# NJU-3DV/Relightable3DGaussian

Measured on AMD Instinct MI355X. Metric: train iters/s, synthetic lego-like 800x800, 300000 Gaussians (stage-2 hot path), higher is better.
Workload: dtype f32; 1 GPU; stage-2 train iteration (fused glue kernels + one-launch Adam): shading fwd/bwd (K=64) + rasterize fwd (S=16) + loss + rasterize bwd + Adam; 1 view/rank/step, 300000 Gaussians, 800x800, num_rendered~1755023; parallelism=dp1

## Files before the change

### include/r3dg_hip.h

```cpp
#ifndef R3DG_HIP_H
#define R3DG_HIP_H

#include <stddef.h>
#include <stdint.h>

#ifdef __cplusplus
extern "C" {
#endif

#define R3DG_OK 0
#define R3DG_EINVAL (-1)
#define R3DG_EHIP (-2)
#define R3DG_EALLOC (-3)

typedef void* (*r3dg_alloc_fn)(void* user, size_t bytes);

const char* r3dg_last_error(void);
int r3dg_release_scratch(void);
int r3dg_version(void);

int r3dg_max_features_forward(void);
int r3dg_max_features_backward(void);

size_t r3dg_geometry_state_bytes(int P);
// ... 293 lines not shown
int r3dg_densify_accumulate(void* stream, int P, const float* d_viewspace_grad, const float* d_normal_grad,
                            const int32_t* d_radii, const float* d_weights, float* d_xyz_gradient_accum,
                            float* d_normal_gradient_accum, float* d_denom, float* d_weights_accum,
                            float* d_max_radii2D,
                            const float* d_skip_flag);

typedef struct r3dg_densify_config {
    int32_t mode;
    int32_t n_split;
    float grad_threshold, grad_normal_threshold, min_opacity, weights_threshold;
    float dense_size, world_size_limit, split_divisor, max_screen_size;
} r3dg_densify_config;

size_t r3dg_densify_temp_bytes(int P);
int r3dg_densify_plan(void* stream, int P, const r3dg_densify_config* config, const float* d_scaling_raw,
                      const float* d_opacity_raw, const float* d_xyz_gradient_accum,
                      const float* d_normal_gradient_accum, const float* d_denom, const float* d_weights_accum,
                      const float* d_max_radii2D, int32_t* d_src_row, int32_t* d_kind, int32_t* d_counts, void* d_temp);

#define R3DG_DENSIFY_MAX_GROUPS 24
#define R3DG_DENSIFY_ROLE_COPY 0
#define R3DG_DENSIFY_ROLE_XYZ 1
#define R3DG_DENSIFY_ROLE_SCALING 2
typedef struct r3dg_densify_group {
    const float* src_param;
    const float* src_exp_avg;
    const float* src_exp_avg_sq;
    float* dst_param;
    float* dst_exp_avg;
    float* dst_exp_avg_sq;
    uint32_t row_floats, role;
} r3dg_densify_group;
int r3dg_densify_gather(void* stream, int rows_out, const int32_t* d_src_row, const int32_t* d_kind, int n_groups,
                        const r3dg_densify_group* groups, const float* d_xyz, const float* d_scaling_raw,
                        const float* d_rotation_raw, const float* d_normal_table, float split_divisor);

int r3dg_reset_opacity(void* stream, int P, float* d_opacity_raw, float* d_exp_avg, float* d_exp_avg_sq);

size_t r3dg_knn_temp_bytes(int P);
int r3dg_knn_dist2(void* stream, int P, const float* d_points, float* d_mean_dist2, void* d_temp);

size_t r3dg_bvh_build_temp_bytes(int P);
int r3dg_bvh_build(void* stream, int P, int32_t* d_nodes, float* d_aabbs, int64_t* d_morton, void* d_temp);
int r3dg_bvh_trace_opacity(void* stream, int64_t num_rays, int num_gaussians, const int32_t* d_nodes, const float* d_aabbs,
                           const float* d_rays_o, const float* d_rays_d, const float* d_means3D,
                           const float* d_covs3D, const float* d_opacities, const float* d_normals,
                           int32_t* d_num_contributes, float* d_rendered_opacity, int32_t* d_stack_overflow);

size_t r3dg_bvh_trace_records_bytes(int num_gaussians);
int r3dg_bvh_pack_traversal(void* stream, int num_gaussians, const int32_t* d_nodes, const float* d_aabbs,
                            const float* d_means3D, const float* d_covs3D, const float* d_opacities,
                            const float* d_normals, void* d_records);
int r3dg_bvh_trace_opacity_packed(void* stream, int64_t num_rays, int num_gaussians, void* d_records, const float* d_rays_o,
                                  const float* d_rays_d, int32_t* d_num_contributes, float* d_rendered_opacity,
                                  int32_t* d_stack_overflow);
int r3dg_bvh_trace_visits(void* stream, int num_gaussians, const void* d_records, uint64_t* node_and_leaf_steps);

int r3dg_bvh_trace_count(void* stream, int64_t num_rays, const int32_t* d_nodes, const float* d_aabbs,
                         const float* d_rays_o, const float* d_rays_d, int32_t* d_num_contributes,
                         int32_t* d_stack_overflow);
int r3dg_bvh_trace_fill(void* stream, int64_t num_rays, const int32_t* d_nodes, const float* d_aabbs,
                        const float* d_rays_o, const float* d_rays_d, const float* d_means3D,
                        const int32_t* d_num_contributes, const int64_t* d_offsets_inclusive, uint64_t* d_keys,
                        int32_t* d_point_list, float* d_position_list, int32_t* d_ray_id_list);

size_t r3dg_sort_temp_bytes(int64_t n);
int r3dg_sort_pairs(void* stream, int64_t n, uint64_t* d_keys_in, uint32_t* d_vals_in, uint64_t* d_keys_out,
                    uint32_t* d_vals_out, int end_bit, void* d_temp);

enum r3dg_option {
    R3DG_OPT_TILE_ORDER = 0,
    R3DG_OPT_CULL,
    R3DG_OPT_TILE_BINNING,
    R3DG_OPT_BINNING_BLOCK_K,
    R3DG_OPT_STAGE_SH_ROWS,
    R3DG_OPT_SHADE_FWD_BLOCKS_PER_CU,
    R3DG_OPT_TRACE_FORMULATION,
    R3DG_OPT_TRACE_REFILL,
    R3DG_OPT_TRACE_NODE_WEIGHT,
    R3DG_OPT_TRACE_LEAF_WEIGHT,
    R3DG_OPT_RESERVE_CUS,
    R3DG_OPT_TRACE_COUNT_VISITS,
    R3DG_OPT_BWD_LEAN,
    R3DG_OPT_COUNT
};
int r3dg_set_option(int option, int value);
int r3dg_get_option(int option, int* value);
void* r3dg_context_create(void);
void r3dg_context_destroy(void* ctx);
int r3dg_context_set_option(void* ctx, int option, int value);
int r3dg_context_make_current(void* ctx, void** previous);
int r3dg_selftest_transpose_reduce(void* stream, int N, int dpp, const float* d_in, float* d_out, int* d_chan,
                                   int* d_owner);

int r3dg_profile_enable(int on);
int r3dg_profile_pause(int paused);
int r3dg_profile_num_stages(void);
const char* r3dg_profile_stage_name(int stage);
int r3dg_profile_read(double* ms_out, int* count_out);

#ifdef __cplusplus
}
#endif
#endif
```

### relightable3dgaussian_amd/_lib.py

```python
import ctypes as C
import threading
import os

_HERE = os.path.dirname(os.path.abspath(__file__))
LIB_PATH = os.environ.get("R3DG_LIB_PATH") or os.path.join(_HERE, "lib", "libr3dg_hip.so")

ALLOC_FN = C.CFUNCTYPE(C.c_void_p, C.c_void_p, C.c_size_t)

_lib = None

_f = C.c_float
_i = C.c_int
_p = C.c_void_p

_SIGNATURES = {
    "r3dg_last_error": (C.c_char_p, []),
    "r3dg_version": (_i, []),
    "r3dg_release_scratch": (_i, []),
    "r3dg_max_features_forward": (_i, []),
    "r3dg_max_features_backward": (_i, []),
    "r3dg_bounded_forward_supported": (_i, [_i, _i]),
    "r3dg_geometry_state_bytes": (C.c_size_t, [_i]),
    "r3dg_image_state_bytes": (C.c_size_t, [_i, _i]),
    "r3dg_binning_state_bytes": (C.c_size_t, [C.c_int64]),
# ... 48 lines not shown
    "r3dg_shade_frs_backward": (_i, [_p, _i, _i] + [_p] * 6 + [_i, _i, _p, _f] + [_p] * 6 + [_i] + [_p] * 10 + [_i, _p]),
    "r3dg_shade_frs_incident_chain": (_i, [_p, _i] + [_p] * 8 + [_f] * 5 + [_i, _f, _p, _i]),
    "r3dg_shade_build_transport": (_i, [_p, _i, _i, _i, _p, _p, _p, _p, _p, _f, _p, _p]),
    "r3dg_shade_forward_transport": (_i, [_p, _i, _i] + [_p] * 9),
    "r3dg_shade_build_split": (_i, [_p, _i, _i] + [_p] * 6 + [_f, _p, _p, _p]),
    "r3dg_shade_env_footprints_bytes": (C.c_size_t, [_i, _i]),
    "r3dg_shade_env_footprints": (_i, [_p, _i, _i, _p, _p]),
    "r3dg_shade_forward_split": (_i, [_p, _i, _i] + [_p] * 11 + [_i, _i, _p]),
    "r3dg_shade_backward": (_i, [_p, _i, _i, _i, _p, _p, _p, _p, _p, _p, _i, _i, _p, _p, _p, _p, _p, _p, _p, _p, _p,
                                 _p, _p]),
    "r3dg_shade_backward_cached": (_i, [_p, _i, _i, _i, _p, _p, _p, _p, _p, _p, _i, _i, _p, _p, _p, _p, _p, _p, _p, _p, _p,
                                        _p, _p, _p, _p, _i]),
    "r3dg_render_equation_forward": (_i, [_p, _i, _i, _i, _i] + [_p] * 8 + [_i] + [_p] * 4),
    "r3dg_render_equation_forward_complex": (_i, [_p, _i, _i, _i, _i] + [_p] * 8 + [_i] + [_p] * 11),
    "r3dg_render_equation_backward": (_i, [_p, _i, _i, _i, _i] + [_p] * 8 + [_i] + [_p] * 11),
    "r3dg_clock_probe": (_i, [_p, _i, _p, _p, C.POINTER(C.c_int)]),
    "r3dg_stage2_activate": (_i, [_p, _i] + [_p] * 17),
    "r3dg_stage2_activate_with": (_i, [_p, _i] + [_p] * 17 + [_i, _p, _p, _p, _i]),
    "r3dg_stage2_pack_features": (_i, [_p, _i] + [_p] * 8),
    "r3dg_stage2_unpack_gradients": (_i, [_p, _i, _p, _p, _f, _p, _p, _p, _p]),
    "r3dg_stage2_activate_backward": (_i, [_p, _i] + [_p] * 24),
    "r3dg_stage2_activate_backward_with": (_i, [_p, _i] + [_p] * 24 + [_i, _i, _p, _p, _p, _f, _p, _p, _i]),
    "r3dg_stage2_loss": (_i, [_p, _i, _i] + [_p] * 8 + [_f, _f, _f] + [_p] * 6 + [_i]),
    "r3dg_stage2_smooth_forward": (_i, [_p, _i, _i] + [_p] * 5 + [_f, _f, _f, _p, _p]),
    "r3dg_stage2_smooth_backward": (_i, [_p, _i, _i] + [_p] * 5 + [_f, _f, _f, _i, _p, _p]),
    "r3dg_stage2_smooth_fused": (_i, [_p, _i, _i] + [_p] * 5 + [_f, _f, _f, _i, _p, _p, _p]),
    "r3dg_stage2_pbr_srgb": (_i, [_p, _i, _i] + [_p] * 5),
    "r3dg_stage2_normals_srgb": (_i, [_p, _i, _i, _p, _f, _f, _f, _f] + [_p] * 8),
    "r3dg_ssim_forward": (_i, [_p, _i, _i, _i, _p, _p, _p, _p]),
    "r3dg_ssim_backward": (_i, [_p, _i, _i, _i, _p, _p, _p, _f, _p]),
    "r3dg_ssim_forward_pair": (_i, [_p, _i, _i, _i] + [_p] * 7),
    "r3dg_ssim_backward_pair": (_i, [_p, _i, _i, _i] + [_p] * 5 + [_f, _f, _p, _p]),
    "r3dg_stage1_pack_features": (_i, [_p, _i, _p, _p, _p, _p]),
    "r3dg_stage1_loss": (_i, [_p, _i, _i] + [_p] * 7 + [_f] * 5 + [_p] * 6),
    "r3dg_stage1_activate_backward": (_i, [_p, _i] + [_p] * 16),
    "r3dg_stage2_env_backward": (_i, [_p, _i, _i, _p, _p, _p, _f, _p, _p, _i]),
    "r3dg_adam_step": (_i, [_p, _i, _p, _f, _f, _f, _i, _f, _p]),
    "r3dg_relight_pack_features": (_i, [_p, _i] + [_p] * 7),
    "r3dg_relight_compose": (_i, [_p, _i, _i, _f, _f, _f, _f, _p, _p, _p, _i, _i] + [_p] * 7),
    "r3dg_densify_accumulate": (_i, [_p, _i] + [_p] * 10),
    "r3dg_densify_temp_bytes": (C.c_size_t, [_i]),
    "r3dg_densify_plan": (_i, [_p, _i] + [_p] * 12),
    "r3dg_densify_gather": (_i, [_p, _i, _p, _p, _i, _p, _p, _p, _p, _p, _f]),
    "r3dg_reset_opacity": (_i, [_p, _i, _p, _p, _p]),
    "r3dg_knn_temp_bytes": (C.c_size_t, [_i]),
    "r3dg_knn_dist2": (_i, [_p, _i, _p, _p, _p]),
    "r3dg_bvh_build_temp_bytes": (C.c_size_t, [_i]),
    "r3dg_bvh_build": (_i, [_p, _i, _p, _p, _p, _p]),
    "r3dg_bvh_trace_opacity": (_i, [_p, C.c_int64, _i, _p, _p, _p, _p, _p, _p, _p, _p, _p, _p, _p]),
    "r3dg_bvh_trace_records_bytes": (C.c_size_t, [_i]),
    "r3dg_bvh_pack_traversal": (_i, [_p, _i] + [_p] * 7),
    "r3dg_bvh_trace_opacity_packed": (_i, [_p, C.c_int64, _i] + [_p] * 6),
    "r3dg_bvh_trace_visits": (_i, [_p, _i, _p, C.POINTER(C.c_uint64)]),
    "r3dg_profile_enable": (_i, [_i]),
    "r3dg_profile_pause": (_i, [_i]),
    "r3dg_profile_num_stages": (_i, []),
    "r3dg_profile_stage_name": (C.c_char_p, [_i]),
    "r3dg_profile_read": (_i, [C.POINTER(C.c_double), C.POINTER(_i)]),
}

EXTRA_SIGNATURES = {}


def lib():
    global _lib
    if _lib is None:
        if not os.path.exists(LIB_PATH):
            raise RuntimeError(
                "libr3dg_hip.so not found at %s -- build it with `python -m relightable3dgaussian_amd.build` "
                "(hipcc, gfx950). There is no CPU fallback." % LIB_PATH)
        import torch
        L = C.CDLL(LIB_PATH)
        sigs = dict(_SIGNATURES)
        sigs.update(EXTRA_SIGNATURES)
        for name, (res, args) in sigs.items():
            fn = getattr(L, name)
            fn.restype = res
            fn.argtypes = args
        _lib = L
    return _lib


OPTIONS = ("TILE_ORDER", "CULL", "TILE_BINNING", "BINNING_BLOCK_K", "STAGE_SH_ROWS", "SHADE_FWD_BLOCKS_PER_CU", "TRACE_FORMULATION",
           "TRACE_REFILL", "TRACE_NODE_WEIGHT", "TRACE_LEAF_WEIGHT", "RESERVE_CUS", "TRACE_COUNT_VISITS", "BWD_LEAN")


def set_option(name, value):
    check(lib().r3dg_set_option(OPTIONS.index(name), int(value)), "set_option(%s)" % name)


_live_lock = threading.Lock()
_live_entries = {}


class OptionContext:

    def __init__(self, **options):
        self._h = lib().r3dg_context_create()
        if self._h is None:
            raise RuntimeError("r3dg_context_create failed")
        self._tls = threading.local()
        for k, v in options.items():
            self.set(k, v)

    def set(self, name, value):
        check(lib().r3dg_context_set_option(self._h, OPTIONS.index(name), int(value)), "context_set_option(%s)" % name)

    def __enter__(self):
        prev = _p()
        check(lib().r3dg_context_make_current(self._h, C.byref(prev)), "context_make_current")
        stack = getattr(self._tls, "prev", None)
        if stack is None:
            stack = self._tls.prev = []
        stack.append(prev.value)
        with _live_lock:
            _live_entries[self._h] = _live_entries.get(self._h, 0) + 1
        return self

    def __exit__(self, *exc):
        check(lib().r3dg_context_make_current(self._tls.prev.pop(), None), "context_make_current")
        with _live_lock:
            n = _live_entries.get(self._h, 0) - 1
            if n > 0:
                _live_entries[self._h] = n
            else:
                _live_entries.pop(self._h, None)
        return False

    def __del__(self):
        try:
            if self._h:
                with _live_lock:
                    busy = _live_entries.get(self._h, 0) > 0
                if not busy:
                    lib().r3dg_context_destroy(self._h)
                self._h = None
        except Exception:
            pass


def get_option(name):
    v = C.c_int(0)
    check(lib().r3dg_get_option(OPTIONS.index(name), C.byref(v)), "get_option(%s)" % name)
    return v.value


def check(status, what):
    if status != 0:
        msg = lib().r3dg_last_error()
        raise RuntimeError("%s failed (%d): %s" % (what, status, msg.decode() if msg else "?"))


def ptr(t):
    if t is None or t.numel() == 0:
        return None
    return t.data_ptr()


def current_stream():
    import torch
    raw = getattr(torch._C, "_cuda_getCurrentRawStream", None)
    if raw is not None:
        return raw(torch._C._cuda_getDevice())
    return torch.cuda.current_stream().cuda_stream


def stream_wait(waiter, signaller):
# ... 23 lines not shown
```

### relightable3dgaussian_amd/csrc/capi_core.hip

```cpp
#include "capi_internal.hpp"

#include <map>
#include <mutex>
#include <new>
#include <tuple>
#include <vector>

namespace r3dg {

static thread_local std::string g_last_error;
void set_error(const std::string& msg) { g_last_error = msg; }

struct OptionRow { int id, def, lo, hi; };
constexpr OptionRow kOptions[] = {
    {R3DG_OPT_TILE_ORDER, 1, 0, 1},
    {R3DG_OPT_CULL, 1, 0, 1},
    {R3DG_OPT_TILE_BINNING, 2, 0, 2},
    {R3DG_OPT_BINNING_BLOCK_K, 2, 1, 4},
    {R3DG_OPT_STAGE_SH_ROWS, 1, 0, 1},
    {R3DG_OPT_SHADE_FWD_BLOCKS_PER_CU, 0, 0, 8},
    {R3DG_OPT_TRACE_FORMULATION, 4, 0, 4},
    {R3DG_OPT_TRACE_REFILL, REFILL_MIN_IDLE, 1, 64},
    {R3DG_OPT_TRACE_NODE_WEIGHT, 1, 1, 15},
    {R3DG_OPT_TRACE_LEAF_WEIGHT, 1, 1, 15},
    {R3DG_OPT_RESERVE_CUS, 0, 0, 128},
    {R3DG_OPT_TRACE_COUNT_VISITS, 0, 0, 1},
    {R3DG_OPT_BWD_LEAN, 1, 0, 1},
};
constexpr bool option_rows_in_enum_order()
{
    for (int i = 0; i < (int)(sizeof(kOptions) / sizeof(kOptions[0])); i++)
        if (kOptions[i].id != i) return false;
    return true;
}
static_assert(sizeof(kOptions) / sizeof(kOptions[0]) == R3DG_OPT_COUNT && option_rows_in_enum_order(),
              "kOptions needs one row per r3dg_option, in the order of the enum");

static bool option_known(int option) { return option >= 0 && option < R3DG_OPT_COUNT; }
static bool option_in_range(int option, int value) { return value >= kOptions[option].lo && value <= kOptions[option].hi; }

struct OptionContext {
    int value[R3DG_OPT_COUNT];
    unsigned int set_mask;
};
static OptionContext g_process_options;
static thread_local const OptionContext* tl_context = nullptr;

int opt(int option)
{
    const OptionContext* c = tl_context;
    if (c != nullptr && ((c->set_mask >> option) & 1u)) return c->value[option];
    return (g_process_options.set_mask >> option) & 1u ? g_process_options.value[option] : kOptions[option].def;
}

namespace {
struct ScratchBuf { void* p = nullptr; size_t cap = 0; };
std::mutex g_scratch_mu;
std::map<std::tuple<int, hipStream_t, int>, ScratchBuf> g_scratch;
}

void* stream_scratch(hipStream_t stream, int slot, size_t bytes)
{
    int dev = 0;
    R3DG_HIP(hipGetDevice(&dev));
    std::lock_guard<std::mutex> lk(g_scratch_mu);
    ScratchBuf& b = g_scratch[std::make_tuple(dev, stream, slot)];
    if (b.cap < bytes) {
        const size_t want = b.p == nullptr ? bytes + bytes / 8 + 4096 : std::max(bytes + 4096, 2 * b.cap);
        if (b.p != nullptr) {
            R3DG_HIP(hipStreamSynchronize(stream));
            R3DG_HIP(hipFree(b.p));
            b.p = nullptr;
            b.cap = 0;
        }
        R3DG_HIP(hipMalloc(&b.p, want));
        b.cap = want;
    }
    return b.p;
}

static void release_all_scratch()
{
    R3DG_HIP(hipDeviceSynchronize());
    {
        std::lock_guard<std::mutex> lk(g_scratch_mu);
        for (auto& kv : g_scratch)
            if (kv.second.p != nullptr) (void)hipFree(kv.second.p);
        g_scratch.clear();
    }
    release_gradient_records();
}

static int g_profiling = 0;
struct EventPair { hipEvent_t a, b; };
static std::vector<EventPair> g_events[ST_COUNT];
static std::mutex g_prof_mutex;

StageTimer::StageTimer(hipStream_t s_, int stage_) : s(s_), stage(stage_), on(g_profiling != 0)
{
    if (on) {
        R3DG_HIP(hipEventCreate(&a));
        R3DG_HIP(hipEventCreate(&b));
        R3DG_HIP(hipEventRecord(a, s));
    }
}
void StageTimer::stop()
{
    if (on) {
        R3DG_HIP(hipEventRecord(b, s));
        std::lock_guard<std::mutex> lk(g_prof_mutex);
// ... 225 lines not shown
```

### relightable3dgaussian_amd/csrc/shading.hip

```cpp
#include "launchers.hpp"
#include <cmath>
#include <cstdlib>
#include <map>
#include <mutex>
#include <stdexcept>
#include <tuple>
#include "wave_reduce.hpp"
#include "shading_math.hpp"

namespace r3dg {

constexpr int SHADE_WAVES = 4;
constexpr int ENV_LDS_MAX = 12288;

__device__ __forceinline__ float fast_acosf(float x)
{
    const float ax = fabsf(x);
    const bool big = ax > 0.5f;
    const float z = big ? 0.5f * (1.0f - ax) : x * x;
    const float s = big ? sqrtf(z) : ax;
    float p = 4.2163199048e-2f;
    p = p * z + 2.4181311049e-2f;
    p = p * z + 4.5470025998e-2f;
    p = p * z + 7.4953002686e-2f;
// ... 1079 lines not shown
                                     const float* normals, const float* viewdirs, const float* incidents, const float* env, int He,
                                     int We, const float* visibility, const float* ray_normals, const float* zsamples,
                                     float uniform_area, const int* invalid_list, int n_invalid, float* out, float* feat)
{
    if (n_invalid <= 0) return;
    const FrsSrc src = {base_color, roughness, normals, viewdirs, ray_normals, nullptr, nullptr, nullptr, visibility, nullptr};
    const size_t smem = ((((size_t)3 * He * We + 3) & ~(size_t)3) + 64 * FRS_LISTED_WAVES) * sizeof(float);
    shade_forward_frs_listed_kernel<<<frs_listed_grid(n_invalid), 64 * FRS_LISTED_WAVES, smem, s>>>(
        n_invalid, invalid_list, K, src, incidents, env, He, We, zsamples, frs_area(uniform_area), out, feat);
    check_launch(s, false, "shade_forward_frs_listed_kernel");
}

const unsigned int* launch_shade_frs_backward_aux(hipStream_t s, int P, const float* g_pbr, const float* g_diff,
                                                  const float* block_absmax, int n_block_absmax, int* gmax_n)
{
    unsigned int* scratch = shade_scratch();
    const unsigned int* gmax = scratch;
    *gmax_n = 1;
    if (block_absmax != nullptr && n_block_absmax > 0) {
        gmax = reinterpret_cast<const unsigned int*>(block_absmax);
        *gmax_n = n_block_absmax;
    } else {
        R3DG_HIP(hipMemsetAsync(scratch, 0, 4, s));
        const int nb = (3 * P + 255) / 256;
        grad_absmax_kernel<<<nb < 256 ? nb : 256, 256, 0, s>>>(3 * P, g_pbr, g_diff, scratch);
    }
    return gmax;
}

void launch_shade_frs_backward_main(hipStream_t s, int P, int K, const float* base_color, const float* roughness,
                                    const float* normals, const float* viewdirs, const float* env, int He, int We,
                                    const float* visibility, float uniform_area, const uint32_t* taps, const float* ray_normals,
                                    const float* tables, const uint8_t* valid, const float* cprime, float* dcp, const float* g_pbr,
                                    const float* g_diff, float* d_base, float* d_rough, float* d_view, float* d_env,
                                    const unsigned int* gmax, int gmax_n)
{
    if (P == 0) return;
    const bool tab_lds = K <= FRS_TAB_LDS_MAX_K;
    const size_t smem = frs_backward_lds_bytes(K, He, We);
    const FrsSrc src = {base_color, roughness, normals, viewdirs, ray_normals, cprime, g_pbr, g_diff, visibility, taps};
    if (tab_lds) {
        const int grid = frs_grid(P, (const void*)shade_backward_frs_kernel<true>, smem);
        shade_backward_frs_kernel<true><<<grid, 64 * FRS_WAVES, smem, s>>>(
            P, K, src, env, He, We, frs_area(uniform_area), tables, valid, d_base, d_rough, d_view, dcp, d_env, gmax, gmax_n);
    } else {
        const int grid = frs_grid(P, (const void*)shade_backward_frs_kernel<false>, smem);
        shade_backward_frs_kernel<false><<<grid, 64 * FRS_WAVES, smem, s>>>(
            P, K, src, env, He, We, frs_area(uniform_area), tables, valid, d_base, d_rough, d_view, dcp, d_env, gmax, gmax_n);
    }
    check_launch(s, false, "shade_backward_frs_kernel");
}

void launch_shade_frs_backward_rotate(hipStream_t s, int P, const float* ray_normals, const float* dcp, float* d_inc,
                                      const uint8_t* valid)
{
    if (P == 0) return;
    frs_rotate_kernel<true><<<(P + 255) / 256, 256, 0, s>>>(P, ray_normals, dcp, d_inc, valid);
    check_launch(s, false, "frs_rotate_kernel");
}

void launch_shade_frs_incident_chain(hipStream_t s, int P, const float* ray_normals, const uint8_t* valid, const float* dcp,
                                     float* d_inc, float* incidents, float* exp_avg, float* exp_avg_sq, float* cprime, float lr,
                                     float lr_tail, float beta1, float beta2, float eps, int step, float grad_scale,
                                     const float* skip_flag, int listed_in_dcprime)
{
    if (P == 0) return;
    const double b1 = 1.0 - pow((double)beta1, (double)step), b2 = 1.0 - pow((double)beta2, (double)step);
    FrsAdam a = {lr, lr_tail, beta1, beta2, eps, (float)b1, (float)(1.0 / sqrt(b2)), grad_scale, 1.f - beta1, 1.f - beta2};
    const size_t lds = 4 * 64 * FRS_CHAIN_LD * sizeof(float);
    frs_incident_chain_kernel<<<(P + 255) / 256, 256, lds, s>>>(P, ray_normals, valid, dcp, d_inc, incidents, exp_avg, exp_avg_sq,
                                                                cprime, a, skip_flag, listed_in_dcprime);
    check_launch(s, false, "frs_incident_chain_kernel");
}

void launch_shade_frs_backward_listed(hipStream_t s, int K, const float* base_color, const float* roughness,
                                      const float* normals, const float* viewdirs, const float* incidents, const float* env, int He,
                                      int We, const float* visibility, const float* ray_normals, const float* zsamples,
                                      float uniform_area, const int* invalid_list, int n_invalid, const float* g_pbr,
                                      const float* g_diff, float* d_base, float* d_rough, float* d_view, float* d_inc, float* d_env,
                                      const unsigned int* gmax, int gmax_n)
{
    if (n_invalid <= 0) return;
    const FrsSrc src = {base_color, roughness, normals, viewdirs, ray_normals, nullptr, g_pbr, g_diff, visibility, nullptr};
    const size_t smem = (3 * (((size_t)3 * He * We + 3) & ~(size_t)3) + 64 * FRS_LISTED_WAVES) * sizeof(float);
    int grid = frs_listed_grid(n_invalid);
    grid = grid > 64 ? 64 + (grid - 64) / 4 : grid;
    if (smem > 65536)
        R3DG_HIP(hipFuncSetAttribute((const void*)shade_backward_frs_listed_kernel, hipFuncAttributeMaxDynamicSharedMemorySize,
                                     (int)smem));
    shade_backward_frs_listed_kernel<<<grid, 64 * FRS_LISTED_WAVES, smem, s>>>(
        n_invalid, invalid_list, K, src, incidents, env, He, We, zsamples, frs_area(uniform_area), d_base, d_rough, d_view, d_inc,
        d_env, gmax, gmax_n);
    check_launch(s, false, "shade_backward_frs_listed_kernel");
}

void launch_shade_build_split(hipStream_t s, int P, int K, const int* perm, const float* normals, const float* incidents,
                              const float* visibility, const float* dirs, const float* zsamples, float uniform_area, float* lt,
                              float* vis_t, float* consts)
{
    if (P == 0) return;
    shade_build_split_kernel<<<(P + 255) / 256, 256, 0, s>>>(P, K, perm, normals, incidents, visibility, dirs, zsamples,
                                                           frs_area(uniform_area), reinterpret_cast<float4*>(lt), vis_t, consts);
    check_launch(s, false, "shade_build_split_kernel");
}

void launch_shade_forward_split(hipStream_t s, int P, int K, const int* perm, const float* base_color, const float* roughness,
                                const float* normals, const float* viewdirs, const float* lt, const float* vis_t,
                                const float* consts, const float* zsamples, const float* tr, const float* env_fp, int He, int We,
                                float* out)
{
    if (P == 0) return;
    const int waves = (P + 63) / 64;
    int parts = (12 * 4 * shade_cus() + waves - 1) / waves;
    parts = parts < 1 ? 1 : (parts > 8 ? 8 : parts);
    int Kp = ((K + parts - 1) / parts + 3) & ~3;
    parts = (K + Kp - 1) / Kp;
    float4* partial = reinterpret_cast<float4*>(stream_scratch(s, 1, (size_t)parts * P * 3 * sizeof(float4)));
    const dim3 grid((P + 255) / 256, parts);
    shade_forward_split_kernel<<<grid, 256, 0, s>>>(P, K, Kp, perm, base_color, roughness, normals, viewdirs,
                                                   reinterpret_cast<const float4*>(lt), vis_t, zsamples, tr,
                                                   reinterpret_cast<const float4*>(env_fp), He, We, partial);
    shade_split_combine_kernel<<<(P + 255) / 256, 256, 0, s>>>(P, K, parts, perm, base_color, partial, consts, out);
    check_launch(s, false, "shade_forward_split_kernel");
}

void launch_shade_env_footprints(hipStream_t s, int He, int We, const float* env, float* fp)
{
    const int n = (He + 1) * (We + 1);
    shade_env_footprints_kernel<<<(n + 255) / 256, 256, 0, s>>>(He, We, env, reinterpret_cast<float4*>(fp));
    check_launch(s, false, "shade_env_footprints_kernel");
}

void launch_shade_build_transport(hipStream_t s, int P, int K, int M, const float* normals, const float* incidents,
                                  const float* visibility, const float* dirs, const float* areas, float uniform_area,
                                  float* radiance_to_transport, float* consts)
{
    if (P == 0) return;
    shade_build_transport_kernel<<<(P + TR_WAVES - 1) / TR_WAVES, 64 * TR_WAVES, 0, s>>>(
        P, K, M, normals, incidents, visibility, dirs, areas, uniform_area, radiance_to_transport, consts);
    check_launch(s, false, "shade_build_transport_kernel");
}

void launch_shade_forward_transport(hipStream_t s, int P, int K, const float* base_color, const float* roughness,
                                    const float* normals, const float* viewdirs, const float* transport, const float* consts,
                                    const float* zsamples, const float* dirs, float* out)
{
    if (P == 0) return;
    shade_forward_transport_kernel<<<(P + TR_WAVES - 1) / TR_WAVES, 64 * TR_WAVES, 0, s>>>(
        P, K, base_color, roughness, normals, viewdirs, transport, consts, zsamples, dirs, out);
    check_launch(s, false, "shade_forward_transport_kernel");
}


}
```

### relightable3dgaussian_amd/csrc/shading_frs.hpp

```cpp
#pragma once
#include "sh_rotation_tables.hpp"

namespace r3dg {

typedef float f32x4 __attribute__((ext_vector_type(4)));

constexpr int FRS_WAVES = 4;
constexpr int FRS_G = 16;
constexpr float FRS_MAX_DEFECT = 2e-5f;
constexpr int FRS_TAB_LDS_MAX_K = 128;

__device__ __forceinline__ void frs_rotation(const float n0, const float n1, const float n2, float (&R)[9])
{
    const float v1 = -n1, v2 = n0, cp = fmaxf(n2 + 1.f, 1e-7f);
    const bool regular = n2 + 1.f > 0.f;
    R[0] = regular ? 1.f + (-v2 * v2) / cp : -1.f;
    R[1] = regular ? v1 * v2 / cp : 0.f;
    R[2] = regular ? v2 : 0.f;
    R[3] = R[1];
    R[4] = regular ? 1.f + (-v1 * v1) / cp : -1.f;
    R[5] = regular ? -v1 : 0.f;
    R[6] = regular ? -v2 : 0.f;
    R[7] = regular ? v1 : 0.f;
    R[8] = regular ? 1.f + (-v2 * v2 - v1 * v1) / cp : -1.f;
// ... 798 lines not shown
            o[1] = make_float4(dcq[1][1], dcq[2][1], dcq[0][2], dcq[1][2]);
            o[2] = make_float4(dcq[2][2], dcq[0][3], dcq[1][3], dcq[2][3]);
        }
    }
    if (fixed) {
        __syncthreads();
        const float inv = 1.0f / fx_scale;
        for (int i = threadIdx.x; i < 3 * ntexel; i += blockDim.x) {
            const long long v64 = s_denv[i];
            if (v64 != 0) atomicAdd(&d_env[i], (float)((double)v64 * (double)inv));
        }
    }
}

constexpr int FRS_LISTED_WAVES = 4;

__device__ __forceinline__ float frs_listed_record(int lane, int g, const FrsSrc& p, const float* __restrict__ incidents)
{
    const float* q = incidents + (size_t)g * 48 + lane;
    if (lane >= 48) q = p.base_color + 3 * (size_t)g + (lane - 48);
    if (lane == 51) q = p.roughness + g;
    if (lane >= 52) q = p.normals + 3 * (size_t)g + (lane - 52);
    if (lane >= 55) q = p.viewdirs + 3 * (size_t)g + (lane - 55);
    if (lane >= 58) q = p.ray_normals + 3 * (size_t)g + (lane - 58);
    return lane < 61 ? *q : 0.f;
}

__device__ __forceinline__ void frs_listed_direction(const float (&R)[9], const float* __restrict__ zsamples, int k, float& dx,
                                                     float& dy, float& dz)
{
    const float zx = zsamples[3 * k], zy = zsamples[3 * k + 1], zz = zsamples[3 * k + 2];
    dx = R[0] * zx + R[1] * zy + R[2] * zz; dy = R[3] * zx + R[4] * zy + R[5] * zz; dz = R[6] * zx + R[7] * zy + R[8] * zz;
    const float len = fmaxf(sqrtf(dx * dx + dy * dy + dz * dz), 1e-12f);
    dx /= len; dy /= len; dz /= len;
}

__global__ void __launch_bounds__(64 * FRS_LISTED_WAVES)
shade_forward_frs_listed_kernel(int n_list, const int* __restrict__ list, int K, FrsSrc src,
                                const float* __restrict__ incidents, const float* __restrict__ env, int He, int We,
                                const float* __restrict__ zsamples, float uniform_area, float* __restrict__ out,
                                float* __restrict__ feat)
{
    extern __shared__ __attribute__((aligned(16))) float s_mem[];
    float* s_env = s_mem;
    const int ntex = 3 * He * We;
    for (int i = threadIdx.x; i < ntex; i += blockDim.x) s_env[i] = env[i];
    __syncthreads();
    const int lane = threadIdx.x & 63, wave = threadIdx.x >> 6;
    float* u = s_mem + ((ntex + 3) & ~3) + wave * 64;
    const float invK = 1.0f / (float)K;
    for (int i = blockIdx.x * FRS_LISTED_WAVES + wave; i < n_list; i += gridDim.x * FRS_LISTED_WAVES) {
        const int g = __builtin_amdgcn_readfirstlane(list[i]);
        u[lane] = frs_listed_record(lane, g, src, incidents);
        GaussFwd G;
        gauss_setup(G, u);
        float R[9];
        frs_rotation(u[58], u[59], u[60], R);
        float v[8] = {0.f, 0.f, 0.f, 0.f, 0.f, 0.f, 0.f, 0.f};
        for (int kb = 0; kb < K; kb += 64) {
            const int k = kb + lane, kc = min(k, K - 1);
            float dx, dy, dz;
            frs_listed_direction(R, zsamples, kc, dx, dy, dz);
            const float vis = src.visibility[(size_t)g * K + kc];
            SampleFwd s;
            shade_sample<true>(s, G, u, 16, dx, dy, dz, vis, uniform_area, nullptr, s_env, nullptr, He, We);
            if (k < K) {
#pragma unroll
                for (int c = 0; c < 3; c++) {
                    v[c] += (G.base[c] / kPi + s.spec) * s.transport[c];
                    v[3 + c] += s.transport[c];
                }
                v[6] += vis;
            }
        }
        const float r = transpose_reduce<8, true>(v);
        const int ch = transposed_channel<8>(lane);
        if (transposed_owner<8>(lane) && ch < 7) {
            out[(size_t)g * SHADE_NOUT + (ch < 6 ? ch : 18)] = r * invK;
            if (feat != nullptr) feat[(size_t)g * 16 + (ch < 3 ? 2 + ch : 9 + ch)] = r * invK;
        }
    }
}

__global__ void __launch_bounds__(64 * FRS_LISTED_WAVES)
shade_backward_frs_listed_kernel(int n_list, const int* __restrict__ list, int K, FrsSrc src,
                                 const float* __restrict__ incidents, const float* __restrict__ env, int He, int We,
                                 const float* __restrict__ zsamples, float uniform_area, float* __restrict__ d_base,
                                 float* __restrict__ d_rough, float* __restrict__ d_view, float* __restrict__ d_inc,
                                 float* __restrict__ d_env, const unsigned int* __restrict__ gmax_bits, int gmax_n)
{
    extern __shared__ __attribute__((aligned(16))) float s_mem[];
    const int ntex = 3 * He * We, ntex4 = (ntex + 3) & ~3;
    float* s_env = s_mem;
    long long* s_denv = reinterpret_cast<long long*>(s_mem + ntex4);
    const unsigned int gmax_word = wave_gmax_bits(gmax_bits, gmax_n);
    const float gmax = __uint_as_float(gmax_word);
    const bool fixed = gmax_usable(gmax_word);
    const float fx_scale = fixed ? 34359738368.0f / gmax : 0.f;
    const float fx_clamp = gmax * 8192.0f;
    for (int i = threadIdx.x; i < ntex; i += blockDim.x) {
        s_env[i] = env[i];
        s_denv[i] = 0;
    }
    __syncthreads();
    const int lane = threadIdx.x & 63, wave = threadIdx.x >> 6;
    float* u = s_mem + 3 * ntex4 + wave * 64;
    const float invK = 1.0f / (float)K;
    for (int i = blockIdx.x * FRS_LISTED_WAVES + wave; i < n_list; i += gridDim.x * FRS_LISTED_WAVES) {
        const int g = __builtin_amdgcn_readfirstlane(list[i]);
        u[lane] = frs_listed_record(lane, g, src, incidents);
        GaussFwd G;
        gauss_setup(G, u);
        float R[9];
        frs_rotation(u[58], u[59], u[60], R);
        float gp[3], gd[3];
#pragma unroll
        for (int c = 0; c < 3; c++) {
            gp[c] = src.g_pbr[3 * (size_t)g + c] * invK;
            gd[c] = src.g_diff[3 * (size_t)g + c] * invK;
        }
        float acc[64];
#pragma unroll
        for (int f = 0; f < 64; f++) acc[f] = 0.f;
        for (int kb = 0; kb < K; kb += 64) {
            const int k = kb + lane, kc = min(k, K - 1);
            float dx, dy, dz;
            frs_listed_direction(R, zsamples, kc, dx, dy, dz);
            const float vis = src.visibility[(size_t)g * K + kc];
            SampleFwd s;
            shade_sample<true>(s, G, u, 16, dx, dy, dz, vis, k < K ? uniform_area : 0.f, nullptr, s_env, nullptr, He, We);
            float gspec = 0.f, dlin[3], dl[3];
#pragma unroll
            for (int c = 0; c < 3; c++) {
                const float dT = gp[c] * (G.base[c] / kPi + s.spec) + gd[c];
                gspec += gp[c] * s.transport[c];
                acc[48 + c] += gp[c] * s.transport[c] / kPi;
                dlin[c] = dT * s.area_ndi;
                dl[c] = s.shsum[c] >= 0.f ? dlin[c] : 0.f;
            }
            if (s.vis != 0.f && s.area_ndi != 0.f) {
                const float ev[3] = {dlin[0] * s.vis, dlin[1] * s.vis, dlin[2] * s.vis};
                const double scale_d = (double)fx_scale;
#pragma unroll
                for (int tt = 0; tt < 4; tt++) {
                    if (s.taps.idx[tt] < 0) continue;
#pragma unroll
                    for (int c = 0; c < 3; c++) {
                        const float val = ev[c] * s.taps.w[tt];
                        if (fixed) {
                            const float cl = __builtin_amdgcn_fmed3f(val, -fx_clamp, fx_clamp);
                            const double dsum = __builtin_fma((double)cl, scale_d, 6755399441055744.0);
                            const unsigned long long bits = (unsigned long long)__double_as_longlong(dsum) - 0x4338000000000000ull;
                            atomicAdd(reinterpret_cast<unsigned long long*>(&s_denv[3 * s.taps.idx[tt] + c]), bits);
                        } else {
                            atomicAdd(&d_env[3 * (size_t)s.taps.idx[tt] + c], val);
                        }
                    }
                }
            }
            const float frac = s.frac0 * G.a2;
            const bool nom_free = s.nomr >= 1e-6f && s.nomr <= 4.f * kPi;
            const float nom = fminf(fmaxf(s.nomr, 1e-6f), 4.f * kPi);
            const float dfrac = gspec / nom;
            const float dnom = nom_free ? -gspec * frac / (nom * nom) : 0.f;
            float da2 = dfrac * s.frac0;
            const float dFMi = dfrac * G.a2 * 0.96f * 0.6931471805599453f * s.p2;
            float dVoH = dFMi * (-2.f * 5.55473f * s.VoH - 6.98316f);
            const float c4 = 4.f * kPi;
            const float dnom0 = dnom * c4 * 2.f * s.nom0 * s.nom1 * s.nom2;
            const float dnom1 = dnom * c4 * s.nom0 * s.nom0 * s.nom2;
            const float dnom2 = dnom * c4 * s.nom0 * s.nom0 * s.nom1;
            float dNoH = dnom0 * 2.f * s.NoH * (G.a2 - 1.f);
            da2 += dnom0 * s.NoH * s.NoH;
            float dNoV = dnom1 * (1.f - G.kk);
            const float dkk = dnom1 * (1.f - G.NoV) + dnom2 * (1.f - s.NoL);
            const float da = dkk / 8.f + da2 * 2.f * G.a;
            acc[51] += dkk * 2.f / 8.f + da * 2.f * G.r;
            if (!(s.rawNoH >= 1e-6f && s.rawNoH <= 1.f)) dNoH = 0.f;
            if (!(s.rawVoH >= 1e-6f && s.rawVoH <= 1.f)) dVoH = 0.f;
            if (!(G.rawNoV >= 1e-6f && G.rawNoV <= 1.f)) dNoV = 0.f;
            float dH[3], dV[3];
#pragma unroll
            for (int c = 0; c < 3; c++) {
                dH[c] = dNoH * G.N[c] + dVoH * G.V[c];
                dV[c] = dVoH * s.Hh[c] + dNoV * G.N[c];
            }
            const float hd = s.Hh[0] * dH[0] + s.Hh[1] * dH[1] + s.Hh[2] * dH[2];
#pragma unroll
            for (int c = 0; c < 3; c++) dV[c] += 0.5f * (dH[c] - s.Hh[c] * hd) / s.ulen;
            const float vd = G.V[0] * dV[0] + G.V[1] * dV[1] + G.V[2] * dV[2];
#pragma unroll
            for (int c = 0; c < 3; c++) acc[52 + c] += (dV[c] - G.V[c] * vd) / G.vlen;
#pragma unroll
            for (int f = 0; f < 48; f++) acc[f] += dl[f % 3] * s.Y[f / 3];
        }
        const float r = transpose_reduce<64, true>(acc);
        const int ch = transposed_channel<64>(lane);
        if (ch < 48) d_inc[(size_t)g * 48 + ch] = r;
        else if (ch < 51) d_base[3 * (size_t)g + (ch - 48)] = r;
        else if (ch == 51) d_rough[g] = r;
        else if (ch < 55) d_view[3 * (size_t)g + (ch - 52)] = r;
    }
    if (fixed) {
// ... 11 lines not shown
```

Baseline: 815.5 iters/s.

## Restructure listed FRS backward prologue and size grid to CU count

The listed FRS shading backward kernel now runs 8 waves per block. Its launch grid is capped at the CU count, or at a new option value, instead of a heuristic. The prologue splits the gmax reduction across the whole block and issues the first Gaussian's record load before staging the environment map, so these latencies overlap. A single block barrier inside the first loop iteration then publishes gmax. The intent is to cut redundant per-wave gmax scans and serialized prologue latency, at the cost of fewer, larger blocks and extra control flow for out-of-range waves.

```diff
diff --git a/include/r3dg_hip.h b/include/r3dg_hip.h
--- a/include/r3dg_hip.h
+++ b/include/r3dg_hip.h
@@ -399,6 +399,7 @@
     R3DG_OPT_RESERVE_CUS,
     R3DG_OPT_TRACE_COUNT_VISITS,
     R3DG_OPT_BWD_LEAN,
+    R3DG_OPT_SHADE_LISTED_GRID_CAP,
     R3DG_OPT_COUNT
 };
 int r3dg_set_option(int option, int value);
diff --git a/relightable3dgaussian_amd/_lib.py b/relightable3dgaussian_amd/_lib.py
--- a/relightable3dgaussian_amd/_lib.py
+++ b/relightable3dgaussian_amd/_lib.py
@@ -154,7 +154,8 @@
 
 
 OPTIONS = ("TILE_ORDER", "CULL", "TILE_BINNING", "BINNING_BLOCK_K", "STAGE_SH_ROWS", "SHADE_FWD_BLOCKS_PER_CU", "TRACE_FORMULATION",
-           "TRACE_REFILL", "TRACE_NODE_WEIGHT", "TRACE_LEAF_WEIGHT", "RESERVE_CUS", "TRACE_COUNT_VISITS", "BWD_LEAN")
+           "TRACE_REFILL", "TRACE_NODE_WEIGHT", "TRACE_LEAF_WEIGHT", "RESERVE_CUS", "TRACE_COUNT_VISITS", "BWD_LEAN",
+           "SHADE_LISTED_GRID_CAP")
 
 
 def set_option(name, value):
diff --git a/relightable3dgaussian_amd/csrc/capi_core.hip b/relightable3dgaussian_amd/csrc/capi_core.hip
--- a/relightable3dgaussian_amd/csrc/capi_core.hip
+++ b/relightable3dgaussian_amd/csrc/capi_core.hip
@@ -26,6 +26,7 @@
     {R3DG_OPT_RESERVE_CUS, 0, 0, 128},
     {R3DG_OPT_TRACE_COUNT_VISITS, 0, 0, 1},
     {R3DG_OPT_BWD_LEAN, 1, 0, 1},
+    {R3DG_OPT_SHADE_LISTED_GRID_CAP, 0, 0, 4096},
 };
 constexpr bool option_rows_in_enum_order()
 {
diff --git a/relightable3dgaussian_amd/csrc/shading.hip b/relightable3dgaussian_amd/csrc/shading.hip
--- a/relightable3dgaussian_amd/csrc/shading.hip
+++ b/relightable3dgaussian_amd/csrc/shading.hip
@@ -1185,13 +1185,14 @@
 {
     if (n_invalid <= 0) return;
     const FrsSrc src = {base_color, roughness, normals, viewdirs, ray_normals, nullptr, g_pbr, g_diff, visibility, nullptr};
-    const size_t smem = (3 * (((size_t)3 * He * We + 3) & ~(size_t)3) + 64 * FRS_LISTED_WAVES) * sizeof(float);
-    int grid = frs_listed_grid(n_invalid);
-    grid = grid > 64 ? 64 + (grid - 64) / 4 : grid;
+    const size_t smem = (3 * (((size_t)3 * He * We + 3) & ~(size_t)3) + 65 * FRS_LISTED_BWD_WAVES) * sizeof(float);
+    const int want = (n_invalid + FRS_LISTED_BWD_WAVES - 1) / FRS_LISTED_BWD_WAVES;
+    const int cap = opt(R3DG_OPT_SHADE_LISTED_GRID_CAP) > 0 ? opt(R3DG_OPT_SHADE_LISTED_GRID_CAP) : shade_cus();
+    const int grid = want < cap ? want : cap;
     if (smem > 65536)
         R3DG_HIP(hipFuncSetAttribute((const void*)shade_backward_frs_listed_kernel, hipFuncAttributeMaxDynamicSharedMemorySize,
                                      (int)smem));
-    shade_backward_frs_listed_kernel<<<grid, 64 * FRS_LISTED_WAVES, smem, s>>>(
+    shade_backward_frs_listed_kernel<<<grid, 64 * FRS_LISTED_BWD_WAVES, smem, s>>>(
         n_invalid, invalid_list, K, src, incidents, env, He, We, zsamples, frs_area(uniform_area), d_base, d_rough, d_view, d_inc,
         d_env, gmax, gmax_n);
     check_launch(s, false, "shade_backward_frs_listed_kernel");
diff --git a/relightable3dgaussian_amd/csrc/shading_frs.hpp b/relightable3dgaussian_amd/csrc/shading_frs.hpp
--- a/relightable3dgaussian_amd/csrc/shading_frs.hpp
+++ b/relightable3dgaussian_amd/csrc/shading_frs.hpp
@@ -904,7 +904,9 @@
     }
 }
 
-__global__ void __launch_bounds__(64 * FRS_LISTED_WAVES)
+constexpr int FRS_LISTED_BWD_WAVES = 8;
+
+__global__ void __launch_bounds__(64 * FRS_LISTED_BWD_WAVES)
 shade_backward_frs_listed_kernel(int n_list, const int* __restrict__ list, int K, FrsSrc src,
                                  const float* __restrict__ incidents, const float* __restrict__ env, int He, int We,
                                  const float* __restrict__ zsamples, float uniform_area, float* __restrict__ d_base,
@@ -915,22 +917,49 @@
     const int ntex = 3 * He * We, ntex4 = (ntex + 3) & ~3;
     float* s_env = s_mem;
     long long* s_denv = reinterpret_cast<long long*>(s_mem + ntex4);
-    const unsigned int gmax_word = wave_gmax_bits(gmax_bits, gmax_n);
-    const float gmax = __uint_as_float(gmax_word);
-    const bool fixed = gmax_usable(gmax_word);
-    const float fx_scale = fixed ? 34359738368.0f / gmax : 0.f;
-    const float fx_clamp = gmax * 8192.0f;
-    for (int i = threadIdx.x; i < ntex; i += blockDim.x) {
-        s_env[i] = env[i];
-        s_denv[i] = 0;
-    }
-    __syncthreads();
-    const int lane = threadIdx.x & 63, wave = threadIdx.x >> 6;
+    const int lane = threadIdx.x & 63, wave = __builtin_amdgcn_readfirstlane(threadIdx.x >> 6);
     float* u = s_mem + 3 * ntex4 + wave * 64;
+    unsigned int* s_gmax = reinterpret_cast<unsigned int*>(s_mem + 3 * ntex4 + 64 * FRS_LISTED_BWD_WAVES);
+    constexpr int NT = 64 * FRS_LISTED_BWD_WAVES;
+    const int tid = threadIdx.x;
+    unsigned int gm = 0u;
+    for (int i0 = tid; i0 < gmax_n; i0 += 4 * NT) {
+        unsigned int b[4];
+#pragma unroll
+        for (int j = 0; j < 4; j++) b[j] = i0 + j * NT < gmax_n ? gmax_bits[i0 + j * NT] & 0x7fffffffu : 0u;
+#pragma unroll
+        for (int j = 0; j < 4; j++) gm = not_finite_bits(b[j]) ? 0x7f800000u : (b[j] > gm ? b[j] : gm);
+    }
+    const int first = blockIdx.x * FRS_LISTED_BWD_WAVES, stride = gridDim.x * FRS_LISTED_BWD_WAVES;
+    int g = __builtin_amdgcn_readfirstlane(list[min(first + wave, n_list - 1)]);
+    float rec = frs_listed_record(lane, g, src, incidents);
+    for (int i0 = tid; i0 < ntex; i0 += 4 * NT) {
+        float e[4];
+#pragma unroll
+        for (int j = 0; j < 4; j++) e[j] = i0 + j * NT < ntex ? env[i0 + j * NT] : 0.f;
+#pragma unroll
+        for (int j = 0; j < 4; j++)
+            if (i0 + j * NT < ntex) {
+                s_env[i0 + j * NT] = e[j];
+                s_denv[i0 + j * NT] = 0;
+            }
+    }
+#pragma unroll
+    for (int o = 32; o > 0; o >>= 1) {
+        const unsigned int other = (unsigned int)__shfl_xor((int)gm, o, 64);
+        gm = other > gm ? other : gm;
+    }
+    if (lane == 0) s_gmax[wave] = gm;
+    bool fixed = false;
+    float fx_scale = 0.f, fx_clamp = 0.f;
     const float invK = 1.0f / (float)K;
-    for (int i = blockIdx.x * FRS_LISTED_WAVES + wave; i < n_list; i += gridDim.x * FRS_LISTED_WAVES) {
-        const int g = __builtin_amdgcn_readfirstlane(list[i]);
-        u[lane] = frs_listed_record(lane, g, src, incidents);
+    for (int base = first; base < n_list; base += stride) {
+        const int i = base + wave;
+        if (base != first) {
+            g = __builtin_amdgcn_readfirstlane(list[min(i, n_list - 1)]);
+            rec = frs_listed_record(lane, g, src, incidents);
+        }
+        u[lane] = rec;
         GaussFwd G;
         gauss_setup(G, u);
         float R[9];
@@ -941,6 +970,17 @@
             gp[c] = src.g_pbr[3 * (size_t)g + c] * invK;
             gd[c] = src.g_diff[3 * (size_t)g + c] * invK;
         }
+        if (base == first) {
+            __syncthreads();
+            unsigned int gmax_word = 0u;
+#pragma unroll
+            for (int w = 0; w < FRS_LISTED_BWD_WAVES; w++) gmax_word = s_gmax[w] > gmax_word ? s_gmax[w] : gmax_word;
+            const float gmax = __uint_as_float(gmax_word);
+            fixed = gmax_usable(gmax_word);
+            fx_scale = fixed ? 34359738368.0f / gmax : 0.f;
+            fx_clamp = gmax * 8192.0f;
+        }
+        if (i >= n_list) continue;
         float acc[64];
 #pragma unroll
         for (int f = 0; f < 64; f++) acc[f] = 0.f;
```

Result: no change. 814.5 iters/s, median of 2 (-0.1%).
